# metno/gridpp

Measured on AMD Instinct MI355X. Metric: grid cells/sec for optimal_interpolation, 4000x4000 grid, 10k obs, higher is better.
Workload: dtype f32 (rho, distances) + f64 (local solve)

## Files before the change

gridpp_amd/__init__.py:

```python
import collections
import ctypes as C

import numpy as np

from . import _capi
from . import _marshal as _m
from ._capi import check, lib
from ._marshal import _empty_like_field, _host_empty, _is_dev, _mem, _ndim, _out_shape, _ptr, _shape, _vec, _wants_f64

__version__ = "0.8.0.dev1+mi355x.r1"

Geodetic, Cartesian = 0, 1
Mean, Min, Median, Max, Quantile, Std, Variance, Sum, Count, RandomChoice, Unknown = 0, 10, 20, 30, 40, 50, 60, 70, 80, 90, -1
MV = np.nan
radius_earth = 6.378137e6


def version():
    return lib().gpp_version().decode()


def set_device(index):
    check(lib().gpp_set_device(int(index)))

# ... 777 lines not shown
        return self._selection(1)

    def weights(self):
        return self._selection(2)


def optimal_interpolation_gain(bgrid, points, pratios, structure, max_points, usable=None):
    if not isinstance(bgrid, (Grid, Points)) or not isinstance(points, Points):
        raise TypeError("bgrid must be a Grid or Points, points a Points")
    if bgrid.get_coordinate_type() != points.get_coordinate_type():
        raise ValueError("Both background and observations points must be of same coordinate type (lat/lon or x/y)")
    max_points = int(max_points)
    if max_points < 1:
        raise ValueError("max_points must be >= 1: a gain holds max_points columns per background point")
    if max_points > _capi.OI_GAIN_MAX_POINTS:
        raise ValueError("max_points must be <= %d (GPP_OI_GAIN_MAX_POINTS)" % _capi.OI_GAIN_MAX_POINTS)
    S = points.size()
    pratios = np.ascontiguousarray(np.asarray(pratios.cpu() if _is_dev(pratios) else pratios), dtype=np.float32)
    if pratios.ndim != 1 or pratios.shape[0] != S:
        raise ValueError("Ratios (%s) and points (%d) size mismatch" % (pratios.shape, S))
    if usable is not None:
        usable = np.ascontiguousarray(np.asarray(usable.cpu() if _is_dev(usable) else usable).astype(bool), dtype=np.uint8)
        if usable.ndim != 1 or usable.shape[0] != S:
            raise ValueError("usable (%s) and points (%d) size mismatch" % (usable.shape, S))
    handle = C.c_void_p()
    check(lib().gpp_oi_gain_create(bgrid._h, points._h, _ptr(pratios), _ptr(usable), _structure(structure), max_points, C.byref(handle)))
    return OiGain(handle, bgrid, S, max_points)


def oi_last_stats():
    s = _capi.gpp_oi_stats()
    check(lib().gpp_oi_last_stats(C.byref(s)))
    return dict(cells=s.cells, cells_updated=s.cells_updated, solves=s.solves, fallback_tiles=s.fallback_tiles, kernel_ms=s.kernel_ms,
                union_kernel_ms=s.union_kernel_ms, fallback_subtiles=s.fallback_subtiles, big_cells=s.big_cells)


def obs_index_axes(points):
    a, b = C.c_int(-1), C.c_int(-1)
    check(lib().gpp_debug_obs_axes(points._h, C.byref(a), C.byref(b)))
    return a.value, b.value


def obs_index_layout(points):
    dims, geom = np.zeros(3, np.int32), np.zeros(3, np.float32)
    check(lib().gpp_debug_obs_index(points._h, _ptr(dims), _ptr(geom), None, 0))
    start = np.zeros(int(dims[0]) * int(dims[1]) + 1, np.int32)
    check(lib().gpp_debug_obs_index(points._h, _ptr(dims), _ptr(geom), _ptr(start), start.size))
    return {"nbx": int(dims[0]), "nby": int(dims[1]), "amin": geom[0], "bmin": geom[1], "inv_s": geom[2], "bin_start": start,
            "device_built": bool(dims[2])}


def _interpolate_levels(entry, igrid, opoints, values, rank_message, pad_empty):
    nd = 2 if isinstance(igrid, Grid) else 1
    f64 = _wants_f64(values)
    values = _m.field(values, f64=f64)
    if pad_empty and not _is_dev(values) and values.size == 0 and values.ndim < nd:
        values = values.reshape((0,) * nd)
    shp = _shape(values)
    if len(shp) not in (nd, nd + 1):
        raise RuntimeError(rank_message)
    levels = len(shp) == nd + 1
    if nd == 2:
        empty = shp[0] == 0 or (levels and shp[1] == 0)
    else:
        empty = levels and shp[0] == 0
    if not empty and tuple(shp[-nd:]) != _out_shape(igrid):
        raise ValueError("Grid size is not the same as values" if nd == 2 else "Points size is not the same as values")
# ... 1534 lines not shown
```

gridpp_amd/_capi.py:

```python
import ctypes as C
import os

_HERE = os.path.dirname(os.path.abspath(__file__))
LIB_PATH = os.environ.get("GPP_LIB") or os.path.join(_HERE, "lib", "libgridpp_hip.so")

GPP_OK, GPP_EINVAL, GPP_ERUNTIME, GPP_ENODEVICE = 0, -1, -2, -3
MEM_HOST, MEM_DEVICE, ASYNC, HOST_F64, Q_HOST = 0, 1, 2, 4, 8
ENSEMBLE_ROW_CAP = 1024
WINDOW_TILE_ROWS, WINDOW_TILE_COLS, WINDOW_FUSED_SPAN = 64, 32, 31
SCORE_TILE_COLS, SCORE_TILE_ROWS, SCORE_FUSED_MAXHW = 64, 32, 16
FSS_TILE_COLS, FSS_TILE_ROWS, FSS_FUSED_MAXHW = 64, 32, 16
POINTWISE_BLOCK, POINTWISE_MAX_BLOCKS = 256, 2048
GAMMA_BLOCK, GAMMA_MAX_BLOCKS = 256, 2048
MO_TILE_ITEMS, MO_GROUP = 2048, 4
OI_GAIN_MAX_POINTS = 62
TRANSFORM_IDENTITY, TRANSFORM_LOG, TRANSFORM_BOXCOX, TRANSFORM_STARTED_BOXCOX = 0, 1, 2, 3
(DIAG_DEWPOINT, DIAG_RELATIVE_HUMIDITY, DIAG_WETBULB, DIAG_PRESSURE, DIAG_SEA_LEVEL_PRESSURE, DIAG_QNH, DIAG_WIND_SPEED,
 DIAG_WIND_DIRECTION) = range(8)


class gpp_structure(C.Structure):
    _fields_ = [("kind", C.c_int), ("h", C.c_float), ("v", C.c_float), ("w", C.c_float), ("min_rho", C.c_float),
                ("kind_v", C.c_int), ("kind_w", C.c_int), ("loc", C.c_float), ("cv_dist", C.c_float), ("flags", C.c_int),
                ("field", C.c_void_p), ("field_v", C.c_void_p), ("field_w", C.c_void_p)]


class gpp_oi_stats(C.Structure):
    _fields_ = [("cells", C.c_longlong), ("cells_updated", C.c_longlong), ("solves", C.c_longlong),
                ("fallback_tiles", C.c_longlong), ("kernel_ms", C.c_float), ("union_kernel_ms", C.c_float), ("fallback_subtiles", C.c_longlong), ("big_cells", C.c_longlong)]


class gpp_ensi_stats(C.Structure):
    _fields_ = [("cells", C.c_longlong), ("condition_passthrough", C.c_longlong), ("real_part_passthrough", C.c_longlong), ("kernel_ms", C.c_float)]


_lib = None
fp = C.POINTER(C.c_float)
ip = C.POINTER(C.c_int)
vp = C.c_void_p

SIGNATURES = {
    "gpp_device_count": [ip],
    "gpp_set_device": [C.c_int],
    "gpp_get_stream": [C.POINTER(vp)],
    "gpp_synchronize": [],
    "gpp_host_alloc": [C.c_size_t, C.POINTER(vp)],
    "gpp_host_free": [vp],
    "gpp_points_create": [vp, vp, vp, vp, C.c_int, C.c_int, C.POINTER(vp)],
    "gpp_grid_create": [vp, vp, vp, vp, C.c_int, C.c_int, C.c_int, C.POINTER(vp)],
    "gpp_points_create_f64": [vp, vp, vp, vp, C.c_int, C.c_int, C.POINTER(vp)],
    "gpp_grid_create_f64": [vp, vp, vp, vp, C.c_int, C.c_int, C.c_int, C.POINTER(vp)],
    "gpp_points_destroy": [vp],
    "gpp_points_size": [vp, ip, ip, ip, ip],
    "gpp_points_get": [vp, C.c_int, vp],
    "gpp_convert_coordinates": [vp, vp, C.c_int, C.c_int, vp, vp, vp],
    "gpp_points_get_neighbours": [vp, C.c_float, C.c_float, C.c_float, C.c_int, vp, vp, C.c_int, ip],
    "gpp_points_get_closest_neighbours": [vp, C.c_float, C.c_float, C.c_int, C.c_int, vp, ip],
    "gpp_points_nearest_neighbour": [vp, vp, vp, C.c_int, C.c_int, vp],
    "gpp_nearest": [vp, vp, vp, vp, C.c_int],
    "gpp_nearest_levels": [vp, vp, vp, C.c_int, vp, C.c_int],
    "gpp_bilinear": [vp, vp, vp, C.c_int, vp, C.c_int],
    "gpp_fill": [vp, vp, vp, vp, C.c_float, C.c_int, vp, C.c_int],
# ... 144 lines not shown
```

gridpp_amd/csrc/oi.hip:

```cpp
#include "oi_common.h"
#include "oi_union.h"

void gpp_launch_union64(const OiArgs& a, unsigned nblocks, bool plain, bool list, hipStream_t stream);
void gpp_launch_union48(const OiArgs& a, unsigned nblocks, bool plain, bool list, hipStream_t stream);
#include <rocprim/rocprim.hpp>
#include <cfloat>
#include <algorithm>
#include <memory>

#pragma clang fp contract(off)

using namespace gpp;

void gpp_free_obs_index(gpp_obs_index* p) { delete p; }

__global__ void k_ix_bins(const float* __restrict__ a, const float* __restrict__ b, int n, float amin, float bmin, float inv_s, int nbx, int nby,
                          int* __restrict__ bin, int* __restrict__ iota) {
    const int i = blockIdx.x * blockDim.x + threadIdx.x;
    if(i >= n) return;
    int bx = (int)floorf((a[i] - amin) * inv_s), by = (int)floorf((b[i] - bmin) * inv_s);
    bx = max(0, min(nbx - 1, bx)); by = max(0, min(nby - 1, by));
    bin[i] = by * nbx + bx;
    iota[i] = i;
}
// ... 1528 lines not shown
    void prepare_runtime() {
        bgrid->to_device();
        ix = gpp_build_obs_index(points);
        if(!ws.e0) { GPP_HIP(hipEventCreate(&ws.e0)); GPP_HIP(hipEventCreate(&ws.e1)); GPP_HIP(hipEventCreate(&ws.eu)); }
        if((mem & GPP_ASYNC) && !g_aslots[0].h) {
            for(int k = 0; k < ASYNC_SLOTS; k++) {
                AsyncSlot& sl = g_aslots[k];
                GPP_HIP(hipHostMalloc((void**)&sl.h, SB * sizeof(unsigned long long), hipHostMallocDefault));
                GPP_HIP(hipEventCreate(&sl.e0)); GPP_HIP(hipEventCreate(&sl.e1)); GPP_HIP(hipEventCreateWithFlags(&sl.ec, hipEventDisableTiming));
            }
            for(int k = 0; k < 2; k++) { GPP_HIP(hipEventCreateWithFlags(&ws.ev_pack[k], hipEventDisableTiming)); GPP_HIP(hipEventCreateWithFlags(&ws.ev_join2[k], hipEventDisableTiming)); }
            (void)stream2(); (void)stream3();
        }
    }
    void fill_args() {
        N = (max_points > 0 && max_points <= 32) ? 32 : 62;
        a.gx = bgrid->d_x.p; a.gy = bgrid->d_y.p; a.gz = bgrid->d_z.p; a.gelev = bgrid->d_elev.p; a.glaf = bgrid->d_laf.p;
        a.bg = f_bg.d; a.bvar = f_bvar.d; a.out = f_out.d; a.out_var = f_var.d;
        a.C = C; a.ny = bgrid->ny; a.nx = bgrid->nx;
        a.tiled2d = (bgrid->nx > 0 && (long)bgrid->ny * bgrid->nx == C) ? 1 : 0;
        a.wshift = 3;
        if(a.tiled2d) {
            a.wshift = gpp_tile_wshift(bgrid);
            const int tw = 1 << a.wshift, th = 64 >> a.wshift;
            a.tiles_x = (a.nx + tw - 1) / tw; a.ntiles = a.tiles_x * ((a.ny + th - 1) / th);
        }
        else { a.tiles_x = 0; a.ntiles = (C + 63) / 64; }
        a.ogeo = ix->d_ogeo.p; a.S = S;
        gpp_scan_geometry(a.s, ix, S, max_points, N);
        a.s.st = gpp_resolve_structure(st);
        gpp_bind_field(a.s.st, st, bgrid, points, ws.cell_idx, ws.obs_idx);
        a.allow_extrap = allow_extrapolation ? 1 : 0;
        a.debug = timing_env("GPP_OI_DEBUG") ? atoi(timing_env("GPP_OI_DEBUG")) : 0;
        a.tile0 = 0; a.tile_n = a.ntiles;
    }
    void plan_kernels() {
        auto odd = [](int k) { return k == GPP_SK_CRESSMAN || k == GPP_SK_SOAR || k == GPP_SK_TOAR; };
        spatial = a.s.st.fh != nullptr;
        use_lu = spatial || (a.s.st.v != 0 && odd(a.s.st.kv)) || (a.s.st.w != 0 && odd(a.s.st.kw)) || path_env("GPP_OI_FORCE_LU");
        plain = a.s.st.kh == GPP_SK_BARNES && a.s.st.kv == GPP_SK_BARNES && a.s.st.kw == GPP_SK_BARNES && !a.s.st.cv;
        pairs_ok = N == 32 && !spatial && (size_t)C * 128 <= PAIR_PARK_MAX && !path_env("GPP_OI_NO_PAIRS");
        memo_hit = memo.points_id == points->serial && memo.h == a.s.st.h && memo.v == a.s.st.v && memo.w == a.s.st.w && memo.kh == a.s.st.kh &&
                   memo.kv == a.s.st.kv && memo.kw == a.s.st.kw && memo.cv == a.s.st.cv && memo.max_points == max_points;
        const bool memo_says_no = memo_hit && memo.declined > 0.5f;
        use_union = !use_lu && (N == 32 || (max_points > 32 && max_points <= 62)) && !memo_says_no && !path_env("GPP_OI_NO_UNION");
        WPB = N == 32 ? UnionCfg<32>::WPB : UnionCfg<64>::WPB;
        big_ok = N == 62;
        sp_union = spatial && plain && N == 32 && !f_var.d && !path_env("GPP_OI_NO_SP_UNION");
    }
    void plan_bands() {
        static_assert(!UnionCfg<32>::persistent<true>(), "the banded host path launches k_oi_union per band of tile rows");
        banded = band_candidate && a.tiled2d && use_union && N == 32 && !path_env("GPP_OI_PAIR_TILES") && a.ntiles / std::max(a.tiles_x, 1) >= BAND_MIN_TILE_ROWS;
        if(band_candidate && !banded) {
            f_bg.bind(background, C, mem);
            f_bvar.bind(bvariance, C, mem);
            a.bg = f_bg.d; a.bvar = f_bvar.d;
        }
        if(!banded) return;
        if(band_f64) { wide_bg.get(C); if(bvariance) wide_bv.get(C); }
        auto pinned = [](const void* p) { hipPointerAttribute_t at; const bool is = hipPointerGetAttributes(&at, p) == hipSuccess && at.type == hipMemoryTypeHost; (void)hipGetLastError(); return is; };
        band_down = pinned(out) && (!out_variance || pinned(out_variance));
        if(band_down && !path_env("GPP_OI_BANDS_COPY_DOWN")) {
            void* dp = nullptr; void* dv = nullptr;
            bool okp = hipHostGetDevicePointer(&dp, out, 0) == hipSuccess && dp != nullptr;
            if(okp && out_variance) okp = hipHostGetDevicePointer(&dv, out_variance, 0) == hipSuccess && dv != nullptr;
            (void)hipGetLastError();
// ... 293 lines not shown
                               (const float*)f_out.d, (const float*)f_var.d, d_patch, d_pv, d_ids);
            GPP_HIP(hipGetLastError());
            GPP_HIP(hipMemcpyAsync(ws.h_patch, d_patch, words * sizeof(float), hipMemcpyDeviceToHost, stream()));
        }
        GPP_HIP(hipStreamSynchronize(stream()));
        GPP_HIP(hipStreamSynchronize(stream3()));
        if(np > 0) {
            const float* const hp = ws.h_patch;
            const float* const hv = f_var.d ? hp + (size_t)np * 64 : nullptr;
            const int* const ids = reinterpret_cast<const int*>(hp + (size_t)np * 64 * (f_var.d ? 2 : 1));
            const int th = 64 >> a.wshift, tw = 1 << a.wshift;
            for(int i = 0; i < np; i++) {
                const int ty = ids[i] / a.tiles_x, tx = ids[i] - ty * a.tiles_x;
                for(int l = 0; l < 64; l++) {
                    const int y = ty * th + (l >> a.wshift), x = tx * tw + (l & (tw - 1));
                    if(y < a.ny && x < a.nx) { out[(size_t)y * a.nx + x] = hp[(size_t)i * 64 + l]; if(hv) out_variance[(size_t)y * a.nx + x] = hv[(size_t)i * 64 + l]; }
                }
            }
        }
    }
    void deliver() {
        if(bands_down_done && !use_lu && !(err & (ERR_SINGULAR | ERR_OVERFLOW))) patch_bands();
        else if(zero_copy_out) GPP_HIP(hipStreamSynchronize(stream()));
        else if(f_out.host || f_var.host) {
            if(bands_down_done) GPP_HIP(hipStreamSynchronize(stream3()));
            f_out.finish(); f_var.finish();
            GPP_HIP(hipStreamSynchronize(stream()));
        }
    }
    void publish_stats() {
        GPP_HIP(hipEventElapsedTime(&g_stats.kernel_ms, ws.e0, ws.e1));
        g_stats.union_kernel_ms = 0;
        if(ran_union || (ran_sp && !sp_failed)) GPP_HIP(hipEventElapsedTime(&g_stats.union_kernel_ms, ws.e0, ws.eu));
        g_stats.cells_updated = 0; g_stats.solves = 0;
        for(int k = 0; k < GPP_NSLOT; k++) { g_stats.cells_updated += (long long)counters[80 + 2 * k]; g_stats.solves += (long long)counters[81 + 2 * k]; }
        if(timing_env("GPP_SCAN_STATS")) fprintf(stderr, "[gpp] scan: %llu candidates iterated, %llu survivor-branch executions, %d tiles\n", counters[2], counters[3], a.ntiles);
#ifdef GPP_UNION_PROFILE
        { const char* nm[24] = {"cell loads", "bbox+init", "phase-1 loads", "rings", "phase 2", "classify", "union records", "P build", "eliminate", "export", "per-lane",
                                "own classify", "B1 wait", "merge", "B2 wait", "B3 wait", "bisection", "bulk evaluations", "end_bulk", "-", "-", "-", "-", "-"};
          const bool two = counters[20 + 24] != 0;
          for(int w = 0; w < 2; w++) {
              double tot = 0; for(int i = 0; i < 24; i++) tot += (double)counters[20 + 24 * w + i];
              if(tot == 0) continue;
              fprintf(stderr, "[gpp] union phases, wave %d (shader clocks per tile, %%):", w); for(int i = 0; i < 19; i++) fprintf(stderr, " %s %.0f (%.1f%%);", nm[i], counters[20 + 24 * w + i] / (double)a.ntiles * (two ? 2 : 1), 100.0 * counters[20 + 24 * w + i] / tot); fprintf(stderr, " total %.0f\n", tot / (double)a.ntiles * (two ? 2 : 1)); } }
#endif
#ifdef GPP_UNION_STATS
        fprintf(stderr, "[gpp] union: fallback reasons: slots %llu, union>40 %llu, extras>12 %llu, layout %llu, per-cell extras>6 %llu; per tile: insertions %.1f, evictions %.1f, candidates evaluated outside the bulk disc %.1f, records loaded in phase 2 %.1f\n",
                                counters[4], counters[5], counters[6], counters[7], counters[8], counters[9] / (double)a.ntiles, counters[10] / (double)a.ntiles, counters[11] / (double)a.ntiles, counters[12] / (double)a.ntiles);
        fprintf(stderr, "[gpp] union: tiles whose slot-ownership masks disagree with the slots: %llu\n", counters[13]);
#endif
        if(timing_env("GPP_SCAN_STATS")) { fprintf(stderr, "[gpp] wave-level insertions per tile histogram:"); for(int i = 0; i < 70; i++) fprintf(stderr, " %d:%llu", i, counters[4 + i]); fprintf(stderr, "\n"); }
    }
};
}

static int oi_full_impl(gpp_points* bgrid, const float* background, const float* bvariance,
                        gpp_points* points, const float* obs, const float* obs_variance,
                        const float* background_at_points, const float* bvariance_at_points,
                        const gpp_structure* st, int max_points, int allow_extrapolation,
                        float* out, float* out_variance, int mem) {
    GPP_TRY
    if(max_points < 0) invalid("max_points must be >= 0");
    if(!bgrid || !points) invalid("grid/points handle is NULL");
    if(bgrid->type != points->type)
        invalid("Both background and observations points must be of same coordinate type (lat/lon or x/y)");
    if(bgrid->n > 0 && (!background || !out)) invalid("background/out is NULL");
    if(points->n > 0 && (!obs || !obs_variance || !background_at_points)) invalid("observation arrays are NULL");
    ensure_device();
// ... 28 lines not shown
    return GPP_OK;
    GPP_CATCH
}

extern "C" int gpp_optimal_interpolation_full(gpp_points* bgrid, const float* background, const float* bvariance,
                                              gpp_points* points, const float* obs, const float* obs_variance,
                                              const float* background_at_points, const float* bvariance_at_points,
                                              const gpp_structure* st, int max_points, int allow_extrapolation,
                                              float* out, float* out_variance, int mem) {
    const bool async_req = (mem & GPP_ASYNC) && (mem & GPP_MEM_DEVICE);
    const size_t before = g_pending.size();
    const int rc = oi_full_impl(bgrid, background, bvariance, points, obs, obs_variance, background_at_points, bvariance_at_points, st, max_points,
                                allow_extrapolation, out, out_variance, mem);
    if(async_req && g_pending.size() == before) {
        PendingOi pc;
        pc.done = true; pc.rc = rc; pc.stats = g_stats;
        if(rc != GPP_OK) pc.msg = gpp_last_error();
        g_pending.push_back(pc);
    }
    return rc;
}

static int complete_pending(PendingOi& pc) {
    GPP_TRY
    if(pc.done) return pc.rc;
    AsyncSlot& sl = g_aslots[pc.slot];
    GPP_HIP(hipEventSynchronize(sl.ec));
    const int* const hi = reinterpret_cast<const int*>(sl.h);
    const int err = hi[0], n_new = hi[1], left = hi[3];
    if(err == 0 && n_new == 0 && !(pc.skip_k_oi && left > 0)) {
        pc.stats.fallback_tiles = pc.n_remembered; pc.stats.fallback_subtiles = left;
        GPP_HIP(hipEventElapsedTime(&pc.stats.kernel_ms, sl.e0, sl.e1));
        pc.stats.union_kernel_ms = pc.stats.kernel_ms;
        pc.stats.cells_updated = 0; pc.stats.solves = 0;
        const unsigned long long* const c = sl.h + 8;
        for(int k = 0; k < GPP_NSLOT; k++) { pc.stats.cells_updated += (long long)c[80 + 2 * k]; pc.stats.solves += (long long)c[81 + 2 * k]; }
        pc.done = true; pc.rc = GPP_OK;
        return GPP_OK;
    }
    pc.done = true;
    pc.rc = oi_full_impl(pc.bgrid, pc.background, pc.bvariance, pc.points, pc.obs, pc.obs_variance, pc.background_at_points, pc.bvariance_at_points, &pc.st,
                         pc.max_points, pc.allow_extrapolation, pc.out, pc.out_variance, pc.mem);
    pc.stats = g_stats;
    if(pc.rc != GPP_OK) pc.msg = gpp_last_error();
    return pc.rc;
    GPP_CATCH
}
extern "C" int gpp_wait(void) {
    GPP_TRY
    if(g_pending.empty()) invalid("gpp_wait: no asynchronous call is pending");
    PendingOi pc = g_pending.front();
    g_pending.erase(g_pending.begin());
    const int rc = complete_pending(pc);
    g_stats = pc.stats;
    if(rc != GPP_OK) gpp::set_error(pc.msg.c_str());
    return rc;
    GPP_CATCH
}
extern "C" int gpp_pending(int* count) {
    if(!count) return gpp::fail(GPP_EINVAL, "count is NULL");
    *count = (int)g_pending.size();
    return GPP_OK;
}
void gpp_oi_drain_pending() {
    for(PendingOi& pc : g_pending) (void)complete_pending(pc);
}
```

gridpp_amd/csrc/oi_union.h:

```cpp
#pragma once
#include "oi_common.h"

#pragma clang fp contract(off)

struct OiArgs {
    const float *gx, *gy, *gz, *gelev, *glaf, *bg, *bvar;
    float *out, *out_var;
    int C, ny, nx, tiles_x, ntiles, tiled2d;
    int wshift;
    ScanArgs s;
    const float4* ogeo;
    const float4* oaux;
    const float4* saux;
    int S, allow_extrap;
    int* err;
    unsigned long long* counters;
    const int* in_list;
    const int* in_count;
    int* out_list;
    int* out_count;
    int nrun;
    int tile0, tile_n;
    int* tail_count;
    const unsigned char* skip_flags;
    int level;
    const int* parent_count;
    int debug;
    int pair_solo;
    int* big_list;
    int* big_count;
    unsigned long long* big_keys;
    double* big_mat;
    int* huge_list;
    int* huge_count;
    unsigned long long* huge_keys;
    double* huge_mat;
    int huge_kcap, huge_ncap;
    unsigned* pair_sel;
    int* pair_n;
};

#define GPP_NSLOT 512
#define BIG_CAND 8192
#define BIG_N 512
#define BIG_NL 104
#define ERR_OVERFLOW 1
#define ERR_SINGULAR 2

__device__ __forceinline__ int nth_set_bit(unsigned long long mask, int m) {
    int pos = 0;
#pragma unroll
    for(int w = 32; w > 0; w >>= 1) {
        unsigned long long lowmask = (w == 32) ? 0xffffffffull : ((1ull << w) - 1ull);
        int c = __popcll((mask >> pos) & lowmask);
        if(m >= c) { m -= c; pos += w; }
    }
    return pos;
}

#ifdef GPP_UNION_STATS
// ... 121 lines not shown
        if(a.bvar) bvar = a.bvar[cell];
    }
    const bool active = cell >= 0 && d_valid(bg);
    DevStructure st = a.s.st;
    const ScanArgs& sa = a.s;
    float sa_inv_s = sa.inv_s;
    if constexpr(SP) { if(cell >= 0) d_structure_at(st, st.cell_idx ? st.cell_idx[cell] : cell); }
    else if constexpr(!LIST) asm volatile("" : "+s"(st.h), "+s"(st.v), "+s"(st.w), "+s"(st.R), "+s"(sa_inv_s));

    UPROF(0);
    const float R = st.R;
    const int K = sa.K;
    const float h2 = st.h * st.h;
    const bool prune = PLAIN || st.kh == SK_BARNES;
    const float pa = sa.axis_a == 0 ? gx : (sa.axis_a == 1 ? gy : gz);
    const float pb = sa.axis_b == 1 ? gy : (sa.axis_b == 2 ? gz : gx);
    const float amin_t = wave_min(active ? pa : INFINITY), amax_t = wave_max(active ? pa : -INFINITY);
    const float bmin_t = wave_min(active ? pb : INFINITY), bmax_t = wave_max(active ? pb : -INFINITY);
    float emin_t = -INFINITY, emax_t = INFINITY, lmin_t = -INFINITY, lmax_t = INFINITY, kv2 = 0.0f, kw2 = 0.0f;
    if constexpr(PLAIN && !SP) {
        if(d_valid(st.v) && st.v != 0.0f && d_valid(st.h) && st.h != 0.0f) {
            emin_t = wave_min(active ? (d_valid(ge) ? ge : -INFINITY) : INFINITY); emax_t = wave_max(active ? (d_valid(ge) ? ge : INFINITY) : -INFINITY);
            kv2 = (st.h / st.v) * (st.h / st.v) * 0.9999f;
        }
        if(d_valid(st.w) && st.w != 0.0f && d_valid(st.h) && st.h != 0.0f) {
            lmin_t = wave_min(active ? (d_valid(gl) ? gl : -INFINITY) : INFINITY); lmax_t = wave_max(active ? (d_valid(gl) ? gl : INFINITY) : -INFINITY);
            kw2 = (st.h / st.w) * (st.h / st.w) * 0.9999f;
        }
    }
    int cnt = 0;
    unsigned long long mine = 0ull;
    unsigned long long alloc = 0ull;
    bool fb = false;
    constexpr unsigned long long FULL = U_WCAP >= 64 ? ~0ull : ((1ull << (U_WCAP & 63)) - 1ull);
#pragma unroll
    for(int w = 0; w < U_WCAP; ++w) L.rho[w][lane] = INFINITY;
    auto live_mask = [&]() { return wave_or64(mine); };
    auto bulk_own = [&](const bool ok, const int s) {
        const unsigned okm = ok ? ~0u : 0u;
        const unsigned long long bit = 1ull << s;
        mine = ((unsigned long long)d_and_or_sc(okm, (unsigned)(bit >> 32), (unsigned)(mine >> 32)) << 32) | d_and_or_sc(okm, (unsigned)bit, (unsigned)mine);
        cnt -= (int)okm;
    };
    auto worst_slot = [&](float& r0, int& s0, bool& multi) {
        constexpr int NG = U_WCAP / 8;
        float gm[NG];
#pragma unroll
        for(int g = 0; g < NG; ++g) {
            float v[8];
#pragma unroll
            for(int j = 0; j < 8; ++j) v[j] = L.rho[8 * g + j][lane];
            gm[g] = fminf(fminf(fminf(v[0], v[1]), fminf(v[2], v[3])), fminf(fminf(v[4], v[5]), fminf(v[6], v[7])));
        }
        r0 = gm[0];
#pragma unroll
        for(int g = 1; g < NG; ++g) r0 = fminf(r0, gm[g]);
        int gs = 0, ng = 0;
#pragma unroll
        for(int g = 0; g < NG; ++g) { const bool eq = gm[g] == r0; gs = eq ? g : gs; ng += eq ? 1 : 0; }
        const float* const grp = &L.rho[0][lane] + gs * (8 * 64);
        float v[8];
#pragma unroll
        for(int j = 0; j < 8; ++j) v[j] = grp[j * 64];
        int sj = 0, nin = 0;
#pragma unroll
        for(int j = 0; j < 8; ++j) { const bool eq = v[j] == r0; sj = eq ? j : sj; nin += eq ? 1 : 0; }
// ... 95 lines not shown
                anynear |= wave_ballot(ok[q]) & wave_ballot(dist[q] > near_r);
            }
            if(anynear != 0ull) {
#pragma unroll
                for(int q = 0; q < EV; ++q) {
                    const float ox = readlane_f(rec.x, cc[q]), oy = readlane_f(rec.y, cc[q]), oz = readlane_f(rec.z, cc[q]);
                    ok[q] = ok[q] && ox > lox && ox < hix && oy > loy && oy < hiy && oz > loz && oz < hiz;
                }
            }
#pragma unroll
            for(int q = 0; q < EV; ++q) rho[q] = 1.0f;
            if(SP ? wave_ballot(hh) != 0ull : hh) {
#pragma unroll
                for(int q = 0; q < EV; ++q) { const float f = d_barnes_rho_flat(dist[q], rh); rho[q] = hh ? f : 1.0f; }
            }
            if(hvu) {
#pragma unroll
                for(int q = 0; q < EV; ++q) {
                    const float oe = readlane_f(rec.w, cc[q]);
                    const float f = d_barnes_rho_flat(d_valid(oe) ? ge - oe : 0.0f, rv_);
                    rho[q] = (hv && d_valid(oe) && d_valid(ge)) ? rho[q] * f : rho[q];
                }
            }
            if(hwu) {
#pragma unroll
                for(int q = 0; q < EV; ++q) {
                    const float ol = readlane_f(met.x, cc[q]);
                    const float f = d_barnes_rho_flat(d_valid(ol) ? gl - ol : 0.0f, rw_);
                    rho[q] = (hw && d_valid(ol) && d_valid(gl)) ? rho[q] * f : rho[q];
                }
            }
#pragma unroll
            for(int q = 0; q < EV; ++q) rho[q] = ok[q] ? rho[q] : 0.0f;
        };

        auto run_chunk = [&](const float4 rec, const float2 met, const int posv, unsigned long long mask) {
            while(mask != 0ull && !fb) {
                const int c = __builtin_ctzll(mask);
                mask &= mask - 1ull;
                if(UNION_STATS && lane == 0) atomicAdd(&a.counters[11], 1ull);
                if constexpr(!SP) {
                    const float ox = readlane_f(rec.x, c), oy = readlane_f(rec.y, c), oz = readlane_f(rec.z, c);
                    const float dx = ox - gx, dy = oy - gy, dz = oz - gz;
                    float d2 = dx * dx + dy * dy;
                    d2 = d2 + dz * dz;
                    if(wave_ballot(d2 <= thr2) == 0ull) continue;
                }
                const float rho = eval(rec, met, c);
                {
                const unsigned orig = (unsigned)__builtin_amdgcn_readlane(__float_as_int(met.y), c);
                const bool want = rho > 0.0f && (cnt < K || rho > wr || (rho == wr && orig < wo));
                if(wave_ballot(want) != 0ull) {
                    if(alloc == FULL) alloc = live_mask();
                    if(UNION_STATS && lane == 0) atomicAdd(&a.counters[9], 1ull);
                    if(UNION_STATS && wave_ballot(want && cnt >= K) != 0ull && lane == 0) atomicAdd(&a.counters[10], 1ull);
                    if(alloc == FULL) { fb = true; if(UNION_STATS && lane == 0) atomicAdd(&a.counters[4], 1ull); return; }
                    const int slot = __builtin_ctzll(~alloc);
                    alloc |= 1ull << slot;
                    if(lane == 0) { L.wpos[slot] = __builtin_amdgcn_readlane(posv, c); L.worig[slot] = (int)orig; }
                    L.rho[slot][lane] = want ? rho : INFINITY;
                    mine |= want ? (1ull << slot) : 0ull;
                    if(want) {
                        if(cnt < K) {
                            if(cnt == 0 || rho < wr || (rho == wr && orig > wo)) { wr = rho; ws = slot; wo = orig; }
                            cnt++;
                        }
// ... 55 lines not shown
                for(int r = 1; r < nrows; ++r) {
                    const int pr = __builtin_amdgcn_readlane(pre, r);
                    if(lane >= pr) row0 = r;
                    if(lane + 64 >= pr) row1 = r;
                    if(lane + 128 >= pr) row2 = r;
                }
                float4 rec0 = make_float4(NAN, 0, 0, NAN), rec1 = rec0, rec2 = rec0;
                float2 met0 = make_float2(NAN, 0), met1 = met0, met2 = met0;
                int pos0 = 0, pos1 = 0, pos2 = 0;
                float pd0 = INFINITY, pd1 = INFINITY, pd2 = INFINITY;
                {
                    pos0 = __shfl(js, row0) + lane - __shfl(pre, row0);
                    if(lane < total) { rec0 = sa.pgeo[pos0]; met0 = sa.smeta[pos0]; }
                    if(nchunk > 1) {
                        pos1 = __shfl(js, row1) + lane + 64 - __shfl(pre, row1);
                        if(lane + 64 < total) { rec1 = sa.pgeo[pos1]; met1 = sa.smeta[pos1]; }
                    }
                    if(nchunk > 2) {
                        pos2 = __shfl(js, row2) + lane + 128 - __shfl(pre, row2);
                        if(lane + 128 < total) { rec2 = sa.pgeo[pos2]; met2 = sa.smeta[pos2]; }
                    }
                    if(lane < total) pd0 = proj_d2(rec0);
                    if(lane + 64 < total) pd1 = proj_d2(rec1);
                    if(lane + 128 < total) pd2 = proj_d2(rec2);
                }
                UPROF(2);
                constexpr int NR = 4;
                float lo2 = -1.0f;
                int nb = 0;
                bool bulk = true;
                auto end_bulk = [&]() {
                    bulk = false;
                    alloc = nb >= 64 ? ~0ull : ((1ull << nb) - 1ull);
                    float r0;
                    int s0;
                    bool multi;
                    worst_slot(r0, s0, multi);
                    wr = r0; ws = s0;
                    wo = (unsigned)L.worig[s0];
                    if(cnt > 0 && multi) {
                        unsigned bo = 0u;
                        for(unsigned long long mm = alloc; mm; mm &= mm - 1ull) {
                            const int w = __builtin_ctzll(mm);
                            if(L.rho[w][lane] == r0) {
                                const unsigned o = (unsigned)L.worig[w];
                                if(o >= bo) { bo = o; ws = w; }
                            }
                        }
                        wo = bo;
                    }
                    if(prune && cnt == K) { bud2 = -2.0f * h2 * logf(wr) * 1.00002f + 2e-5f * h2; thr2 = fminf(thr2_R, bud2); }
                };
                const int kb = min(K, U_WCAP);
                float tlo = 0.0f;
                {
                    float thi = sa.ring_r0 * sa.ring_r0;
                    const float lim2 = wave_lim2();
                    thi = fminf(thi, lim2);
                    auto count_le = [&](const float t) { return __popcll(wave_ballot(pd0 <= t)) + __popcll(wave_ballot(pd1 <= t)) + __popcll(wave_ballot(pd2 <= t)); };
                    if(count_le(thi) <= kb) tlo = thi;
                    else {
                        for(int it = 0; it < 9; ++it) {
                            const float mid = 0.5f * (tlo + thi);
                            if(count_le(mid) <= kb) tlo = mid; else thi = mid;
                        }
                    }
                }
                UPROF(16);
                for(int ring = -1; ring < NR && !fb; ++ring) {
                    const float hi = d_sqrt_raw(tlo) + (float)(ring + 1) * sa.ring_dr;
                    const float hi2 = ring < 0 ? tlo : ((ring == NR - 1) ? INFINITY : hi * hi);
                    const float lim2 = wave_lim2();
                    if(lim2 < 0.0f || lo2 >= lim2) break;
                    const float B2 = wave_bud2();
                    const unsigned long long m0 = wave_ballot(pd0 > lo2 && pd0 <= hi2 && keep(pd0, rec0, met0, lim2, B2));
                    const unsigned long long m1 = wave_ballot(pd1 > lo2 && pd1 <= hi2 && keep(pd1, rec1, met1, lim2, B2));
                    const unsigned long long m2 = wave_ballot(pd2 > lo2 && pd2 <= hi2 && keep(pd2, rec2, met2, lim2, B2));
                    if(ring >= 0 && bulk) { UPROF(17); end_bulk(); UPROF(18); }
                    for(int k = 0; k < nchunk && !fb; ++k) {
                        const float4 rec = k == 0 ? rec0 : (k == 1 ? rec1 : rec2);
                        const float2 met = k == 0 ? met0 : (k == 1 ? met1 : met2);
                        const int posv = k == 0 ? pos0 : (k == 1 ? pos1 : pos2);
                        const unsigned long long mk = k == 0 ? m0 : (k == 1 ? m1 : m2);
                        if(GPP_DBG(a, 8)) continue;
                        if(bulk) {
                            if((mk >> lane) & 1ull) {
                                const int slot = nb + __popcll(mk & ((1ull << lane) - 1ull));
                                L.wpos[slot] = posv;
                                L.worig[slot] = __float_as_int(met.y);
                            }
                            if constexpr(PLAIN && EV > 1) {
                                for(unsigned long long mm = mk; mm != 0ull;) {
                                    int cc[EV], n = 0;
#pragma unroll
                                    for(int q = 0; q < EV; ++q) {
                                        cc[q] = mm != 0ull ? __builtin_ctzll(mm) : cc[0];
                                        n += mm != 0ull ? 1 : 0;
                                        mm &= mm - 1ull;
                                    }
                                    float rho[EV];
                                    eval_n(rec, met, cc, rho);
#pragma unroll
                                    for(int q = 0; q < EV; ++q) {
                                        if(q < n) {
                                            const bool ok = rho[q] > 0.0f;
                                            L.rho[nb][lane] = ok ? rho[q] : INFINITY;
                                            bulk_own(ok, nb);
                                            nb++;
                                        }
                                    }
                                }
                            }
                            else
                            for(unsigned long long mm = mk; mm != 0ull; mm &= mm - 1ull) {
                                const int c = __builtin_ctzll(mm);
                                const float rho = eval(rec, met, c);
                                const bool ok = rho > 0.0f;
                                L.rho[nb][lane] = ok ? rho : INFINITY;
                                bulk_own(ok, nb);
                                nb++;
                            }
                        }
                        else run_chunk(rec, met, posv, mk);
                    }
// ... 762 lines not shown
                    const double rs = rsqrt_nr(valid ? sii : 1.0);
                    il[i] = rs;
                    qv[i] = gq * rs;
                    tv[i] = dq * rs;
                    if(valid) {
                        inc = __builtin_fma(qv[i], tv[i], inc);
                        if(want_var) a00 = __builtin_fma(qv[i], qv[i], a00);
                        if(!a.allow_extrap) {
                            const float de = __int_as_float(LS.worig[ai]);
                            maxInc = fmaxf(maxInc, de); minInc = fminf(minInc, de);
                        }
                    }
                }
            }
        }
        }
        }
        UPROF(10);
        if(cnt > 0) {
            float increment = (float)inc;
            if(!a.allow_extrap) {
                if(maxInc > 0 && increment > maxInc) increment = maxInc;
                else if(maxInc < 0 && increment > 0) increment = maxInc;
                else if(minInc < 0 && increment < minInc) increment = minInc;
                else if(minInc > 0 && increment < 0) increment = minInc;
            }
            res_out = bg + increment;
            res_var = (float)((double)bvar * (1.0 - a00));
        }
        if(wave_ballot(bad && cnt > 0) != 0ull && lane == 0) atomicOr(a.err, ERR_SINGULAR);
        if(lane == 0 && a.counters) {
            unsigned long long* cs = a.counters + 80 + 2 * (blockIdx.x % GPP_NSLOT);
            atomicAdd(&cs[0], (unsigned long long)__popcll(upd));
            if(solver) atomicAdd(&cs[1], 1ull);
        }
    }
#ifdef GPP_UNION_PROFILE
    if(lane < 24) atomicAdd(&a.counters[20 + 24 * pw + lane], (unsigned long long)L.prof[lane]);
#endif
    if(cell >= 0) {
        a.out[cell] = res_out;
        if(a.out_var) a.out_var[cell] = res_var;
    }
}

template <bool PLAIN, bool LIST, int NC, bool SP = false>
__global__ __launch_bounds__(64 * UnionCfg<NC>::WPB, NC == 64 ? 1 : ((NC == 32 && PLAIN && !SP) ? 3 : 2)) void k_oi_union(OiArgs a) {
    constexpr int WPB = UnionCfg<NC>::WPB;
    __shared__ UnionLds<NC> s_u[WPB];
    if constexpr(PLAIN) { d_exptab_fill<64 * WPB>(); __syncthreads(); }
    const int wid = threadIdx.x >> 6, lane = threadIdx.x & 63;
    if constexpr(LIST) {
        int tile = blockIdx.x * WPB + wid, sub = -1;
        int shift = 0;
        const int nlist = *a.in_count;
        const bool whole = nlist > 0 && a.in_list[0] < 0;
        const bool forward = a.level != 3 && (whole || (a.level == 1 ? nlist > a.ntiles / 2 : nlist > 2 * *a.parent_count));
        if(forward) {
            for(int i = blockIdx.x * (64 * WPB) + threadIdx.x; i < nlist; i += gridDim.x * (64 * WPB)) {
                const int e = a.in_list[i];
                a.out_list[atomicAdd(a.out_count, 1)] = (a.level == 1) ? ~e : e;
            }
            return;
        }
        if(a.level == 3) {
            if(16 * nlist > (int)gridDim.x * WPB || tile >= 16 * nlist) return;
            sub = tile & 15; tile = a.in_list[tile >> 4]; shift = 2;
// ... 84 lines not shown
```

include/gridpp_hip.h:

```cpp
#ifndef GRIDPP_HIP_H
#define GRIDPP_HIP_H

#include <stddef.h>
#ifdef __cplusplus
extern "C" {
#endif

#define GPP_OK 0
#define GPP_EINVAL -1
#define GPP_ERUNTIME -2
#define GPP_ENODEVICE -3

#define GPP_MEM_HOST 0
#define GPP_MEM_DEVICE 1
#define GPP_ASYNC 2
#define GPP_Q_HOST 8
#define GPP_HOST_F64 4

#define GPP_GEODETIC 0
#define GPP_CARTESIAN 1

#define GPP_MEAN 0
#define GPP_MIN 10
#define GPP_MEDIAN 20
// ... 245 lines not shown
int gpp_wind_direction(const float* xwind, const float* ywind, long long n, float* out, int mem);
#define GPP_TRANSFORM_IDENTITY 0
#define GPP_TRANSFORM_LOG 1
#define GPP_TRANSFORM_BOXCOX 2
#define GPP_TRANSFORM_STARTED_BOXCOX 3
int gpp_transform(const float* in, long long n, int kind, int backward, float p0, float p1, float* out, int mem);
#define GPP_DIAG_DEWPOINT 0
#define GPP_DIAG_RELATIVE_HUMIDITY 1
#define GPP_DIAG_WETBULB 2
#define GPP_DIAG_PRESSURE 3
#define GPP_DIAG_SEA_LEVEL_PRESSURE 4
#define GPP_DIAG_QNH 5
#define GPP_DIAG_WIND_SPEED 6
#define GPP_DIAG_WIND_DIRECTION 7
int gpp_diagnostic_scalar(int which, const float* args, int nargs, float* out);
int gpp_transform_scalar(float value, int kind, int backward, float p0, float p1, float* out);

#define GPP_GAMMA_BLOCK 256
#define GPP_GAMMA_MAX_BLOCKS 2048
int gpp_gamma_inv(const float* levels, const float* shape, const float* scale, long long n, float* out, int mem);
int gpp_gamma_transform(const float* in, long long n, int backward, float shape, float scale, float tolerance, float* out, int mem);
int gpp_gamma_inv_scalar(float level, float shape, float scale, float* out);
int gpp_gamma_transform_scalar(float value, int backward, float shape, float scale, float tolerance, float* out);

typedef struct gpp_oi_stats {
    long long cells;
    long long cells_updated;
    long long solves;
    long long fallback_tiles;
    float kernel_ms;
    float union_kernel_ms;
    long long fallback_subtiles;
    long long big_cells;
} gpp_oi_stats;
int gpp_oi_last_stats(gpp_oi_stats* stats);
int gpp_debug_obs_axes(gpp_points* points, int* axis_a, int* axis_b);
int gpp_debug_obs_index(gpp_points* points, int* dims, float* geom, int* bin_start, int cap);

int gpp_wait(void);
int gpp_pending(int* count);

#define GPP_OI_GAIN_MAX_POINTS 62
typedef struct gpp_oi_gain gpp_oi_gain;
int gpp_oi_gain_create(gpp_points* bgrid, gpp_points* points, const float* pratios, const unsigned char* usable,
                       const gpp_structure* structure, int max_points, gpp_oi_gain** gain);
int gpp_oi_gain_apply(gpp_oi_gain* gain, const float* background, int ne, const float* pobs, int pobs_per_field, const float* pbackground,
                      int allow_extrapolation, float* out, int mem);
int gpp_oi_gain_variance(gpp_oi_gain* gain, const float* bvariance, float* out, int mem);
int gpp_oi_gain_info(const gpp_oi_gain* gain, long long* cells, int* stations, int* max_points, long long* bytes, int* largest_selection);
int gpp_oi_gain_selection(gpp_oi_gain* gain, int* counts, int* indices, double* weights, int mem);
int gpp_oi_gain_destroy(gpp_oi_gain* gain);

typedef struct gpp_downscale_plan gpp_downscale_plan;
int gpp_downscale_plan_create(gpp_points* igrid, gpp_points* to, int downscaler, gpp_downscale_plan** plan);
int gpp_downscale_plan_apply(gpp_downscale_plan* plan, const float* values, int nt, float* out, int mem);
int gpp_downscale_plan_apply_cube(gpp_downscale_plan* plan, const float* values, int ne, float* out, int mem);
int gpp_downscale_plan_simple_gradient(gpp_downscale_plan* plan, const float* values, int nt, float elev_gradient, float* out, int mem);
int gpp_downscale_plan_full_gradient(gpp_downscale_plan* plan, const float* values, int nt, const float* elev_gradient,
                                     const float* laf_gradient, float* out, int mem);
int gpp_downscale_plan_simple_gradient_cube(gpp_downscale_plan* plan, const float* values, int ne, float elev_gradient, float* out, int mem);
int gpp_downscale_plan_full_gradient_cube(gpp_downscale_plan* plan, const float* values, int ne, const float* elev_gradient, int elev_members,
                                          const float* laf_gradient, int laf_members, float* out, int mem);
int gpp_downscale_plan_probability(gpp_downscale_plan* plan, const float* values, int ne, const float* threshold, int comparison_operator,
                                   float* out, int mem);
int gpp_downscale_plan_mask_threshold(gpp_downscale_plan* plan, const float* ivalues_true, const float* ivalues_false,
                                      const float* threshold_values, int ne, const float* threshold, int comparison_operator, int statistic,
// ... 10 lines not shown
```

Baseline: 4.234 billion.

## Certify whole-wave bulk observation sets to skip per-lane cutoff and vertical checks

Adds a wave-level geometric certificate for plain Barnes structures without vertical or land-area-fraction terms. If every candidate chunk is provably within every active cell's localization radius, using the third-axis extent and near radius, the bulk loop evaluates rho with a simplified distance-only path. It also sets cnt and mine directly to all collected observations instead of classifying each one. This trades an extra wave reduction and ballot per wave for cheaper per-observation evaluation. It adds a new counter packed into the high bits of the solve atomic and an environment switch to disable it.

```diff
diff --git a/gridpp_amd/__init__.py b/gridpp_amd/__init__.py
--- a/gridpp_amd/__init__.py
+++ b/gridpp_amd/__init__.py
@@ -833,7 +833,7 @@
     s = _capi.gpp_oi_stats()
     check(lib().gpp_oi_last_stats(C.byref(s)))
     return dict(cells=s.cells, cells_updated=s.cells_updated, solves=s.solves, fallback_tiles=s.fallback_tiles, kernel_ms=s.kernel_ms,
-                union_kernel_ms=s.union_kernel_ms, fallback_subtiles=s.fallback_subtiles, big_cells=s.big_cells)
+                union_kernel_ms=s.union_kernel_ms, fallback_subtiles=s.fallback_subtiles, big_cells=s.big_cells, bulk_certified=s.bulk_certified)
 
 
 def obs_index_axes(points):
diff --git a/gridpp_amd/_capi.py b/gridpp_amd/_capi.py
--- a/gridpp_amd/_capi.py
+++ b/gridpp_amd/_capi.py
@@ -27,7 +27,8 @@
 
 class gpp_oi_stats(C.Structure):
     _fields_ = [("cells", C.c_longlong), ("cells_updated", C.c_longlong), ("solves", C.c_longlong),
-                ("fallback_tiles", C.c_longlong), ("kernel_ms", C.c_float), ("union_kernel_ms", C.c_float), ("fallback_subtiles", C.c_longlong), ("big_cells", C.c_longlong)]
+                ("fallback_tiles", C.c_longlong), ("kernel_ms", C.c_float), ("union_kernel_ms", C.c_float), ("fallback_subtiles", C.c_longlong), ("big_cells", C.c_longlong),
+                ("bulk_certified", C.c_longlong)]
 
 
 class gpp_ensi_stats(C.Structure):
diff --git a/gridpp_amd/csrc/oi.hip b/gridpp_amd/csrc/oi.hip
--- a/gridpp_amd/csrc/oi.hip
+++ b/gridpp_amd/csrc/oi.hip
@@ -1584,6 +1584,7 @@
         gpp_bind_field(a.s.st, st, bgrid, points, ws.cell_idx, ws.obs_idx);
         a.allow_extrap = allow_extrapolation ? 1 : 0;
         a.debug = timing_env("GPP_OI_DEBUG") ? atoi(timing_env("GPP_OI_DEBUG")) : 0;
+        a.no_bulk_cert = path_env("GPP_OI_NO_BULK_CERT") ? 1 : 0;
         a.tile0 = 0; a.tile_n = a.ntiles;
     }
     void plan_kernels() {
@@ -1943,8 +1944,11 @@
         GPP_HIP(hipEventElapsedTime(&g_stats.kernel_ms, ws.e0, ws.e1));
         g_stats.union_kernel_ms = 0;
         if(ran_union || (ran_sp && !sp_failed)) GPP_HIP(hipEventElapsedTime(&g_stats.union_kernel_ms, ws.e0, ws.eu));
-        g_stats.cells_updated = 0; g_stats.solves = 0;
-        for(int k = 0; k < GPP_NSLOT; k++) { g_stats.cells_updated += (long long)counters[80 + 2 * k]; g_stats.solves += (long long)counters[81 + 2 * k]; }
+        g_stats.cells_updated = 0; g_stats.solves = 0; g_stats.bulk_certified = 0;
+        for(int k = 0; k < GPP_NSLOT; k++) {
+            g_stats.cells_updated += (long long)counters[80 + 2 * k];
+            g_stats.solves += (long long)(counters[81 + 2 * k] & 0xffffffffull); g_stats.bulk_certified += (long long)(counters[81 + 2 * k] >> 32);
+        }
         if(timing_env("GPP_SCAN_STATS")) fprintf(stderr, "[gpp] scan: %llu candidates iterated, %llu survivor-branch executions, %d tiles\n", counters[2], counters[3], a.ntiles);
 #ifdef GPP_UNION_PROFILE
         { const char* nm[24] = {"cell loads", "bbox+init", "phase-1 loads", "rings", "phase 2", "classify", "union records", "P build", "eliminate", "export", "per-lane",
@@ -2039,9 +2043,12 @@
         pc.stats.fallback_tiles = pc.n_remembered; pc.stats.fallback_subtiles = left;
         GPP_HIP(hipEventElapsedTime(&pc.stats.kernel_ms, sl.e0, sl.e1));
         pc.stats.union_kernel_ms = pc.stats.kernel_ms;
-        pc.stats.cells_updated = 0; pc.stats.solves = 0;
+        pc.stats.cells_updated = 0; pc.stats.solves = 0; pc.stats.bulk_certified = 0;
         const unsigned long long* const c = sl.h + 8;
-        for(int k = 0; k < GPP_NSLOT; k++) { pc.stats.cells_updated += (long long)c[80 + 2 * k]; pc.stats.solves += (long long)c[81 + 2 * k]; }
+        for(int k = 0; k < GPP_NSLOT; k++) {
+            pc.stats.cells_updated += (long long)c[80 + 2 * k];
+            pc.stats.solves += (long long)(c[81 + 2 * k] & 0xffffffffull); pc.stats.bulk_certified += (long long)(c[81 + 2 * k] >> 32);
+        }
         pc.done = true; pc.rc = GPP_OK;
         return GPP_OK;
     }
diff --git a/gridpp_amd/csrc/oi_union.h b/gridpp_amd/csrc/oi_union.h
--- a/gridpp_amd/csrc/oi_union.h
+++ b/gridpp_amd/csrc/oi_union.h
@@ -26,6 +26,7 @@
     int level;
     const int* parent_count;
     int debug;
+    int no_bulk_cert;
     int pair_solo;
     int* big_list;
     int* big_count;
@@ -213,6 +214,7 @@
     unsigned long long mine = 0ull;
     unsigned long long alloc = 0ull;
     bool fb = false;
+    bool cert = false;
     constexpr unsigned long long FULL = U_WCAP >= 64 ? ~0ull : ((1ull << (U_WCAP & 63)) - 1ull);
 #pragma unroll
     for(int w = 0; w < U_WCAP; ++w) L.rho[w][lane] = INFINITY;
@@ -374,6 +376,24 @@
             }
 #pragma unroll
             for(int q = 0; q < EV; ++q) rho[q] = ok[q] ? rho[q] : 0.0f;
+        };
+
+        auto eval_cert_n = [&](const float4& rec, const int (&cc)[EV], float (&rho)[EV]) {
+            float dist[EV];
+#pragma unroll
+            for(int q = 0; q < EV; ++q) {
+                const float ox = readlane_f(rec.x, cc[q]), oy = readlane_f(rec.y, cc[q]), oz = readlane_f(rec.z, cc[q]);
+                const float dx = ox - gx, dy = oy - gy, dz = oz - gz;
+                float d2 = dx * dx + dy * dy;
+                d2 = d2 + dz * dz;
+                dist[q] = d_sqrt_cr(d2);
+            }
+#pragma unroll
+            for(int q = 0; q < EV; ++q) rho[q] = 1.0f;
+            if(hh) {
+#pragma unroll
+                for(int q = 0; q < EV; ++q) rho[q] = d_barnes_rho_flat(dist[q], rh);
+            }
         };
 
         auto run_chunk = [&](const float4 rec, const float2 met, const int posv, unsigned long long mask) {
@@ -495,6 +515,7 @@
                 auto end_bulk = [&]() {
                     bulk = false;
                     alloc = nb >= 64 ? ~0ull : ((1ull << nb) - 1ull);
+                    if(cert) { cnt = active ? nb : 0; mine = active ? alloc : 0ull; }
                     float r0;
                     int s0;
                     bool multi;
@@ -529,6 +550,24 @@
                         }
                     }
                 }
+                if constexpr(PLAIN && EV > 1 && !SP && !PAIR) {
+                    if(!hvu && !hwu && !a.no_bulk_cert) {
+                        const int ax3 = 3 - sa.axis_a - sa.axis_b;
+                        const float pc = ax3 == 0 ? gx : (ax3 == 1 ? gy : gz);
+#define third(rec) (ax3 == 0 ? (rec).x : (ax3 == 1 ? (rec).y : (rec).z))
+                        const float cmin_t = wave_min(active ? pc : INFINITY), cmax_t = wave_max(active ? pc : -INFINITY);
+                        float lim = __int_as_float(__builtin_amdgcn_readfirstlane(__float_as_int(wave_min(active ? near_r : INFINITY))));
+                        if(hh) lim = fminf(lim, 12.0f * fabsf(st.h));
+                        lim *= 0.99f;
+                        const float lim2c = lim * lim;
+                        auto far = [&](const float rc, const float pd) __attribute__((always_inline)) {
+                            const float p = d_sqrt_raw(pd) * 1.01f + rad, t = fmaxf(fabsf(rc - cmin_t), fabsf(rc - cmax_t));
+                            return pd <= tlo && !((p * p + t * t) * 1.01f <= lim2c);
+                        };
+                        cert = lim > 0.0f && wave_ballot(far(third(rec0), pd0) || far(third(rec1), pd1) || far(third(rec2), pd2)) == 0ull && wave_ballot(active && !(lim <= near_r)) == 0ull;
+                    }
+                }
+#undef third
                 UPROF(16);
                 for(int ring = -1; ring < NR && !fb; ++ring) {
                     const float hi = d_sqrt_raw(tlo) + (float)(ring + 1) * sa.ring_dr;
@@ -553,6 +592,27 @@
                                 L.worig[slot] = __float_as_int(met.y);
                             }
                             if constexpr(PLAIN && EV > 1) {
+                                if(cert) {
+                                    for(unsigned long long mm = mk; mm != 0ull;) {
+                                        int cc[EV], n = 0;
+#pragma unroll
+                                        for(int q = 0; q < EV; ++q) {
+                                            cc[q] = mm != 0ull ? __builtin_ctzll(mm) : cc[0];
+                                            n += mm != 0ull ? 1 : 0;
+                                            mm &= mm - 1ull;
+                                        }
+                                        float rho[EV];
+                                        eval_cert_n(rec, cc, rho);
+#pragma unroll
+                                        for(int q = 0; q < EV; ++q) {
+                                            if(q < n) {
+                                                L.rho[nb][lane] = active ? rho[q] : INFINITY;
+                                                nb++;
+                                            }
+                                        }
+                                    }
+                                }
+                                else
                                 for(unsigned long long mm = mk; mm != 0ull;) {
                                     int cc[EV], n = 0;
 #pragma unroll
@@ -1381,7 +1441,7 @@
         if(lane == 0 && a.counters) {
             unsigned long long* cs = a.counters + 80 + 2 * (blockIdx.x % GPP_NSLOT);
             atomicAdd(&cs[0], (unsigned long long)__popcll(upd));
-            if(solver) atomicAdd(&cs[1], 1ull);
+            if(solver) atomicAdd(&cs[1], 1ull + (cert ? 1ull << 32 : 0ull));
         }
     }
 #ifdef GPP_UNION_PROFILE
diff --git a/include/gridpp_hip.h b/include/gridpp_hip.h
--- a/include/gridpp_hip.h
+++ b/include/gridpp_hip.h
@@ -301,6 +301,7 @@
     float union_kernel_ms;
     long long fallback_subtiles;
     long long big_cells;
+    long long bulk_certified;
 } gpp_oi_stats;
 int gpp_oi_last_stats(gpp_oi_stats* stats);
 int gpp_debug_obs_axes(gpp_points* points, int* axis_a, int* axis_b);
```

Measured after the change: 4.411 billion (median of 6 runs). 1.04x the previous value.
